# lpylpy0514/VitTracker

Measured on AMD Instinct MI355X. Metric: track() frames/sec per GPU, vit_48_h32, 128px search / 64px template, higher is better.
Workload: dtype f32

## Files before the change

### vittracker_amd/csrc/vt_blocks.h

```cpp
#pragma once
#include <type_traits>
#include "vt_common.h"
#include "vt_bf3.h"

namespace vtb {

constexpr int C = 48;
constexpr int NC = C / 16;
constexpr int HID = 4 * C;
constexpr int NH = HID / 16;
constexpr float LN_EPS = 1e-5f;

constexpr int O_LN1G = 0;
constexpr int O_LN1B = O_LN1G + C;
constexpr int O_WQKV = O_LN1B + C;
constexpr int O_BQKV = O_WQKV + 9 * NC * 256;
constexpr int O_WPROJ = O_BQKV + 3 * C;
constexpr int O_BPROJ = O_WPROJ + NC * NC * 256;
constexpr int O_LN2G = O_BPROJ + C;
constexpr int O_LN2B = O_LN2G + C;
constexpr int O_W1 = O_LN2B + C;
constexpr int O_B1 = O_W1 + NH * NC * 256;
constexpr int O_W2 = O_B1 + HID;
constexpr int O_B2 = O_W2 + NC * NH * 256;
// ... 113 lines not shown
        opa(0, a[0]);
#pragma unroll
        for (int c = 0; c < NCHUNK; ++c) {
            if (c + 1 < NCHUNK) opa(c + 1, a[(c + 1) & 1]);
            if constexpr (SHARED_IS_B) mfma4_shared_b(a[c & 1], ops(c), acc);
            else mfma4_shared_a(ops(c), a[c & 1], acc);
        }
    }
}

template <int NT, int NW, int TPW, bool WLDS, bool BAL = false, bool ZC = false, bool BF3 = false, bool A3 = false>
__global__ __launch_bounds__(NW * 64, (NW == 5 && !WLDS) ? 3 : 1) void blocks_kernel(const float* __restrict__ tokens,
                                                         const float* __restrict__ params,
                                                         float* __restrict__ feat,
                                                         float* __restrict__ resid,
                                                         int len_z, int depth_total, int nblocks,
                                                         int dbg_skip_tile,
                                                         unsigned long long* __restrict__ stamps,
                                                         float* __restrict__ zcache,
                                                         int zcache_mode,
                                                         const float* __restrict__ params3,
                                                         unsigned* __restrict__ vlscr) {
    static_assert(NW * TPW >= NT, "tiles must be covered");
    constexpr bool BF3L = BF3 && WLDS, BF3G = BF3 && !WLDS;
    static_assert(!BF3L || (BAL && 2 * NT * NC >= W3_FC2_TILES - WBUF_TILES), "BF3 with staging: written for the balanced frame form; fc2's third output tile is staged in the K / V area");
    static_assert(!BAL || (WLDS && TPW == 1 && NW == 2 * (NT - 1)), "balanced variant: NT-1 owners + NT-1 guests");
    static_assert(!A3 || BF3, "A3: written for the three-piece forms");
    constexpr bool VP3 = A3 && BF3L;
    constexpr bool VP2L = A3 && BF3G;
    constexpr int KP_T16 = W3_FC1_OT16, VP_PAIRS = NT / 2, VP_T16 = VP_PAIRS * 3 * 64 + (NT & 1) * 3 * 32;
    constexpr int KV_UNITS = A3 ? NT * KP_T16 + (VP3 ? NC * VP_T16 : NC * NT * 64) : 2 * NT * NC * 64;
    constexpr int L = NT * 16;
    constexpr int NOWN = BAL ? NT - 1 : NT;
    constexpr int GT = NT - 1;
    extern __shared__ __attribute__((aligned(16))) float lds[];
    f4* Kimg = reinterpret_cast<f4*>(lds);
    f4* Vimg = Kimg + (A3 ? NT * KP_T16 : NT * NC * 64);
    opnd* const Ko = reinterpret_cast<opnd*>(Kimg);
    opnd* const Vo = reinterpret_cast<opnd*>(Vimg);
    f4* Wa = Kimg + KV_UNITS;
    constexpr int WA_TILES = BF3L ? W3_FC1_TILES : WBUF_TILES;
    f4* Wb = Wa + WA_TILES * 64;
    float* Sp = reinterpret_cast<float*>(WLDS ? Wb + WBUF_TILES * 64 : Wa);
    f4* const Gx = reinterpret_cast<f4*>(Sp + small_floats(depth_total));
    f4* Qg = A3 ? Wb + W3_PROJ_TILES * 64 : Gx;
    f4* Pg = Qg + (A3 ? KP_T16 : NC * 64);
    f4* Dg = A3 ? Gx : Pg + 4 * NC * 64;
    float* Mg = reinterpret_cast<float*>(A3 ? Pg + 4 * NC * 64 : Dg + NC * 64);
    int* gflag = A3 ? reinterpret_cast<int*>(Dg + NC * 64) : reinterpret_cast<int*>(Mg + 4 * 2 * 64);
    f4* Pg2 = A3 ? Wa + W3_QKV_TILES * 64 : Pg;
    static_assert(!A3 || (W3_PROJ_TILES * 64 + KP_T16 + 4 * NC * 64 + 4 * 2 * 64 / 4 <= WBUF_TILES * 64 && W3_QKV_TILES * 64 + 4 * NC * 64 <= W3_FC1_TILES * 64),
                  "A3: the exchange areas fit behind proj's / qkv's image");

    const int b = blockIdx.x;
    const int lane = threadIdx.x & 63;
    const int w = __builtin_amdgcn_readfirstlane(threadIdx.x >> 6);
    const int tok = lane & 15, q = lane >> 4;
    const int g = w - (NT - 1);
    const float scale = 0.14433756729740643f;
    constexpr float SCALE_LOG2E = 0.14433756729740643f * 1.4426950408889634f;
    const int guest_prio = dbg_skip_tile == -3 ? 0 : 1;
    const bool fine = dbg_skip_tile == -2 || dbg_skip_tile <= -100;
    if (dbg_skip_tile <= -100) dbg_skip_tile = -100 - dbg_skip_tile;
    int nstamp = 0;
    auto stamp = [&]() {
        if (stamps != nullptr) {
            unsigned long long t;
            asm volatile("s_memtime %0\n\ts_waitcnt lgkmcnt(0)" : "=s"(t)::"memory");
            if (lane == 0) stamps[((size_t)b * NW + w) * 64 + nstamp] = t;
            ++nstamp;
        }
    };
    auto fstamp = [&]() { if (fine) stamp(); };
    stamp();
    auto stage_img = [&](f4* dst, int off, int ntiles, int blk_of) {
        if constexpr (VT_IS_F16)
            stage_tiles(dst, reinterpret_cast<const float*>(reinterpret_cast<const _Float16*>(params3) + (size_t)blk_of * BLOCK_STRIDE + off), (ntiles + 1) / 2, w, NW, lane);
        else
            stage_tiles(dst, params + (size_t)blk_of * BLOCK_STRIDE + off, ntiles, w, NW, lane);
    };
    if constexpr (BF3L) stage_tiles(Wa, params3 + (W3_FC1_TILES + W3_FC2_TILES) * 256, W3_QKV_TILES, w, NW, lane);
    else if constexpr (WLDS) stage_img(Wa, O_WQKV, 9 * NC, 0);
    for (int i = threadIdx.x; 4 * i < small_floats(depth_total); i += NW * 64)
        st4(Sp + 4 * i, ld4(params + small_src(4 * i, depth_total)));

    f4 x[TPW][NC];
#pragma unroll
    for (int i = 0; i < TPW; ++i) {
        const int T = w + NW * i;
        if (T < NOWN && T != dbg_skip_tile) {
            const float* src = tokens + ((size_t)b * L + 16 * T + tok) * C + 4 * q;
#pragma unroll
            for (int c = 0; c < NC; ++c) x[i][c] = ld4(src + 16 * c);
        }
    }
    f4 x4[NC];
    if constexpr (BAL) {
        if (w >= NOWN) {
            const float* src = tokens + ((size_t)b * L + 16 * GT + tok) * C + 4 * q;
#pragma unroll
            for (int c = 0; c < NC; ++c) x4[c] = ld4(src + 16 * c);
        }
        if (threadIdx.x == 0) *gflag = 0;
        if (w >= NOWN && guest_prio > 0) __builtin_amdgcn_s_setprio(2);
    }
    barrier_publish<WLDS>();

    const int lane_k = lane;
    for (int blk = 0; blk < nblocks; ++blk) {
        int lane_s = lane_k;
        if constexpr (BF3) asm volatile("" : "+v"(lane_s));
        const int lane = lane_s, tok = lane & 15, q = lane >> 4;
        const float* __restrict__ P = params + (size_t)blk * BLOCK_STRIDE;
        const float* S = Sp + blk * SMALL_STRIDE;
        const opnd* const Po = VT_IS_F16 ? reinterpret_cast<const opnd*>(reinterpret_cast<const _Float16*>(params3) + (size_t)blk * BLOCK_STRIDE)
                                         : reinterpret_cast<const opnd*>(P);
        const opnd* const Wa_o = reinterpret_cast<const opnd*>(Wa);
        const opnd* const Wb_o = reinterpret_cast<const opnd*>(Wb);
        auto w_qkv = [&](int t) { return WLDS ? Wa_o[t * 64 + lane] : wimg_o(Po + O_WQKV / 4, t, lane); };
        auto w_proj = [&](int t) { return WLDS ? Wb_o[t * 64 + lane] : wimg_o(Po + O_WPROJ / 4, t, lane); };
        auto w_fc1 = [&](int t) { return WLDS ? Wa_o[t * 64 + lane] : wimg_o(Po + O_W1 / 4, t, lane); };
        auto w_fc2 = [&](int t) { return WLDS ? Wb_o[t * 64 + lane] : wimg_o(Po + O_W2 / 4, t, lane); };
        const float* __restrict__ P3 = BF3 ? params3 + (size_t)blk * BLOCK3_STRIDE : nullptr;
        constexpr int PROJ_TILES = NC * NC;
        using vt3::u32x2;
        using vt3::u32x4;
        int lane3 = lane;
        if constexpr (BF3) asm volatile("" : "+v"(lane3));
        const auto Wa3 = BF3L ? lds_lane_base<u32x4>(Wa, 16u * lane3) : nullptr;
        const auto Wa3h = BF3L ? lds_lane_base<u32x2>(Wa, 192u * 16u + 8u * lane3) : nullptr;
        const auto Wb3 = BF3L ? lds_lane_base<u32x4>(Wb, 16u * lane3) : nullptr;
        const auto Wk3 = BF3L ? lds_lane_base<u32x4>(Kimg, 16u * lane3) : nullptr;
        auto w1_load3 = [&](int t, u32x4 (&a0)[3], u32x2 (&a2)[3]) {
#pragma unroll
            for (int pc = 0; pc < 3; ++pc) {
                a0[pc] = Wa3[t * W3_FC1_OT16 + pc * 64];
                a2[pc] = Wa3h[t * W3_FC1_OT16 * 2 + pc * 64];
            }
        };
        auto w2_load3 = [&](int p, u32x4 (&a)[NC][3]) {
#pragma unroll
            for (int ot = 0; ot < NC; ++ot)
#pragma unroll
                for (int pc = 0; pc < 3; ++pc)
                    a[ot][pc] = ot < 2 ? Wb3[((ot * (NH / 2) + p) * 3 + pc) * 64] : Wk3[(p * 3 + pc) * 64];
// ... 64 lines not shown
            }
        };
        auto store_v3 = [&](int T, int ot, f4 r) {
            u32x2 pv[3];
            vt3::split3(r, pv[0], pv[1], pv[2]);
            u32x2* base = reinterpret_cast<u32x2*>(Kimg + NT * KP_T16 + ot * VP_T16);
            if ((NT & 1) && T == NT - 1) {
#pragma unroll
                for (int pc = 0; pc < 3; ++pc) base[VP_PAIRS * 3 * 64 * 2 + pc * 64 + lane3] = pv[pc];
            } else {
#pragma unroll
                for (int pc = 0; pc < 3; ++pc) base[(((T >> 1) * 3 + pc) * 64 + lane3) * 2 + (T & 1)] = pv[pc];
            }
        };
        constexpr int VL_BLK_U4 = NC * VP_PAIRS * 64;
        u32x4* const vl_blk = VP2L ? reinterpret_cast<u32x4*>(vlscr) + ((size_t)b * depth_total + blk) * VL_BLK_U4 : nullptr;
        auto store_v2l = [&](int T, int ot, f4 r) {
            u32x2 pv[3];
            vt3::split3(r, pv[0], pv[1], pv[2]);
            const int pp = T >> 1, hf = T & 1;
#pragma unroll
            for (int pc = 0; pc < 2; ++pc) reinterpret_cast<u32x2*>(Vimg)[((((ot * VP_PAIRS + pp) * 2 + pc) * 64) + lane3) * 2 + hf] = pv[pc];
            reinterpret_cast<u32x2*>(vl_blk)[(((ot * VP_PAIRS + pp) * 64) + lane3) * 2 + hf] = pv[2];
        };
        if constexpr (A3 && BF3L) {
            stage_tiles(Wb, P3 + (W3_FC1_TILES + W3_FC2_TILES + W3_QKV_TILES) * 256, W3_PROJ_TILES, w, NW, lane, blk == 0);
        } else if constexpr (BF3L) {
            stage_tiles(Wb, P + O_WPROJ, PROJ_TILES, w, NW, lane, blk == 0);
        } else if constexpr (WLDS) stage_img(Wb, O_WPROJ, NC * NC, blk);

        f4 qr[TPW][NC];
#pragma unroll
        for (int i = 0; i < TPW; ++i) {
            const int T = w + NW * i;
            const bool z_tile = ZC && blk == 0 && 16 * T < len_z;
            int lane_z = lane;
            if constexpr (ZC) asm volatile("" : "+v"(lane_z));
            f4* const zc = reinterpret_cast<f4*>(zcache) + (((size_t)b * (len_z >> 4) + T) * 3 * NC) * 64 + lane_z;
            if (VT_BLK_OWNERS && T < NOWN && T != dbg_skip_tile && z_tile && zcache_mode == 2) {
#pragma unroll
                for (int ot = 0; ot < NC; ++ot) {
                    qr[i][ot] = zc[ot * 64];
                    if constexpr (VP3) store_v3(T, ot, zc[(2 * NC + ot) * 64]);
                    else if constexpr (VP2L) store_v2l(T, ot, zc[(2 * NC + ot) * 64]);
                    else Vo[(ot * NT + T) * 64 + lane] = to_opnd(zc[(2 * NC + ot) * 64]);
                    if constexpr (!A3) Ko[(T * NC + ot) * 64 + lane] = to_opnd(zc[(NC + ot) * 64]);
                }
                if constexpr (A3) {
                    f4 kr[NC];
#pragma unroll
                    for (int ot = 0; ot < NC; ++ot) kr[ot] = zc[(NC + ot) * 64];
                    store_k3(Kimg + T * KP_T16, kr);
                }
            } else if (VT_BLK_OWNERS && T < NOWN && T != dbg_skip_tile) {
                f4 h[NC];
                layer_norm_plain(x[i], h);
                fstamp();
                if constexpr (BF3) {
                    u32x4 hb[3];
                    u32x2 hc[3];
                    split_h3(h, hb, hc);
                    const u32x4* const Gq = reinterpret_cast<const u32x4*>(P3) + (W3_FC1_TILES + W3_FC2_TILES) * 64;
                    const u32x2* const Gqh = reinterpret_cast<const u32x2*>(Gq);
                    auto wq_load3 = [&](int t, u32x4 (&a0)[3], u32x2 (&a2)[3]) {
                        if constexpr (BF3L) w1_load3(t, a0, a2);
                        else {
#pragma unroll
                            for (int pc = 0; pc < 3; ++pc) {
                                a0[pc] = Gq[t * W3_FC1_OT16 + pc * 64 + lane3];
                                a2[pc] = Gqh[(t * W3_FC1_OT16 + 192) * 2 + pc * 64 + lane3];
                            }
                        }
                    };
                    u32x4 a0[2][3];
                    u32x2 a2[2][3];
                    auto bias_q = [&](int t) { return t < 2 * NC ? ld4(S + S_BQKV + 16 * t + 4 * q) : splat4(S[S_BQKV + 2 * C + 16 * (t % NC) + tok]); };
                    f4 bias[2];
                    f4 kr[NC];
                    wq_load3(0, a0[0], a2[0]);
                    bias[0] = bias_q(0);
#pragma unroll
                    for (int t = 0; t < 3 * NC; ++t) {
                        if (t + 1 < 3 * NC) {
                            wq_load3(t + 1, a0[(t + 1) & 1], a2[(t + 1) & 1]);
                            bias[(t + 1) & 1] = bias_q(t + 1);
                        }
                        const int ot = t % NC;
// ... 26 lines not shown
                        [&](int c, opnd (&a)[2 * NC]) {
#pragma unroll
                            for (int ot = 0; ot < 2 * NC; ++ot) a[ot] = w_qkv(ot * NC + c);
                        },
                        [&](int c) { return h[c]; }, acc);
#pragma unroll
                    for (int ot = 0; ot < NC; ++ot) {
                        qr[i][ot] = acc[ot];
                        Ko[(T * NC + ot) * 64 + lane] = to_opnd(acc[NC + ot]);
                        if (z_tile && zcache_mode == 1) { zc[ot * 64] = acc[ot]; zc[(NC + ot) * 64] = acc[NC + ot]; }
                    }
                }
                fstamp();
                {
                    f4 acc[NC];
#pragma unroll
                    for (int ot = 0; ot < NC; ++ot) acc[ot] = splat4(S[S_BQKV + 2 * C + 16 * ot + tok]);
                    gemm_stage<NC, NC, false, WLDS>(
                        [&](int c, opnd (&bw)[NC]) {
#pragma unroll
                            for (int ot = 0; ot < NC; ++ot) bw[ot] = w_qkv((2 * NC + ot) * NC + c);
                        },
                        [&](int c) { return h[c]; }, acc);
#pragma unroll
                    for (int ot = 0; ot < NC; ++ot) {
                        Vo[(ot * NT + T) * 64 + lane] = to_opnd(acc[ot]);
                        if (z_tile && zcache_mode == 1) zc[(2 * NC + ot) * 64] = acc[ot];
                    }
                }
                }
            }
        }
        if constexpr (BAL) {
            if (BF3L && VT_BLK_GUESTS && w >= NOWN && g < 3) {
                f4 h[NC];
                layer_norm_plain(x4, h);
                u32x4 hb[3];
                u32x2 hc[3];
                split_h3(h, hb, hc);
                u32x4 a0[NC][3];
                u32x2 a2[NC][3];
#pragma unroll
                for (int j = 0; j < NC; ++j) w1_load3(NC * g + j, a0[j], a2[j]);
                f4 r[NC];
                if (g < 2) {
                    f4 bias[NC];
#pragma unroll
                    for (int j = 0; j < NC; ++j) bias[j] = ld4(S + S_BQKV + 16 * (g * NC + j) + 4 * q);
                    __builtin_amdgcn_sched_barrier(0);
#pragma unroll
                    for (int j = 0; j < NC; ++j) r[j] = tile48(std::false_type{}, a0[j], a2[j], hb, hc, bias[j]);
                    if constexpr (A3) {
                        store_k3(g == 0 ? Qg : Kimg + GT * KP_T16, r);
                    } else {
#pragma unroll
                        for (int j = 0; j < NC; ++j) {
                            if (g == 0) Qg[j * 64 + lane] = r[j];
                            else Ko[(GT * NC + j) * 64 + lane] = to_opnd(r[j]);
                        }
                    }
                } else {
                    f4 bias[NC];
#pragma unroll
                    for (int j = 0; j < NC; ++j) bias[j] = splat4(S[S_BQKV + 2 * C + 16 * j + tok]);
                    __builtin_amdgcn_sched_barrier(0);
#pragma unroll
                    for (int j = 0; j < NC; ++j) r[j] = tile48(std::true_type{}, a0[j], a2[j], hb, hc, bias[j]);
#pragma unroll
                    for (int j = 0; j < NC; ++j) {
                        if constexpr (A3) store_v3(GT, j, r[j]);
                        else Vo[(j * NT + GT) * 64 + lane] = to_opnd(r[j]);
                    }
                }
            } else if (VT_BLK_GUESTS && w >= NOWN && g < 3) {
                f4 h[NC];
                layer_norm_plain(x4, h);
                f4 acc[NC];
                if (g < 2) {
#pragma unroll
                    for (int ot = 0; ot < NC; ++ot) acc[ot] = ld4(S + S_BQKV + 16 * (g * NC + ot) + 4 * q);
                    gemm_stage<NC, NC, true, true>(
                        [&](int c, opnd (&a)[NC]) {
#pragma unroll
                            for (int ot = 0; ot < NC; ++ot) a[ot] = w_qkv((g * NC + ot) * NC + c);
                        },
                        [&](int c) { return h[c]; }, acc);
#pragma unroll
                    for (int ot = 0; ot < NC; ++ot) {
                        if (g == 0) Qg[ot * 64 + lane] = acc[ot];
                        else Ko[(GT * NC + ot) * 64 + lane] = to_opnd(acc[ot]);
                    }
                } else {
#pragma unroll
                    for (int ot = 0; ot < NC; ++ot) acc[ot] = splat4(S[S_BQKV + 2 * C + 16 * ot + tok]);
                    gemm_stage<NC, NC, false, true>(
                        [&](int c, opnd (&bw)[NC]) {
#pragma unroll
                            for (int ot = 0; ot < NC; ++ot) bw[ot] = w_qkv((2 * NC + ot) * NC + c);
                        },
                        [&](int c) { return h[c]; }, acc);
#pragma unroll
                    for (int ot = 0; ot < NC; ++ot) Vo[(ot * NT + GT) * 64 + lane] = to_opnd(acc[ot]);
                }
            }
        }
        stamp();
        if constexpr (VP2L) asm volatile("s_waitcnt vmcnt(0)" ::: "memory");
        barrier_publish<WLDS>();
        stamp();
        if constexpr (BF3L) {
            stage_tiles(Wa, P3, W3_FC1_TILES, w, NW, lane, blk == 0);
        } else if constexpr (WLDS) stage_img(Wa, O_W1, NH * NC, blk);
        const bool last_skip_z = (blk == depth_total - 1) && (resid == nullptr);
#pragma unroll
        for (int i = 0; i < TPW; ++i) {
            const int T = w + NW * i;
            if (A3 && VT_BLK_OWNERS && T < NOWN && T != dbg_skip_tile && !(last_skip_z && 16 * T < len_z)) {
                constexpr int TW[6] = {2, 0, 1, 1, 0, 0}, TX[6] = {0, 2, 1, 0, 1, 0};
                u32x4 qb[3];
                u32x2 qc[3];
                split_h3(qr[i], qb, qc);
                f4 s[NT];
                float m0 = -3.0e38f, m1 = -3.0e38f;
                {
                    constexpr int NB = VP3 ? 2 : 1;
                    u32x4 a0[NB][3];
                    u32x2 a2[NB][3];
                    if (NB == 2) k_load3(0, a0[0], a2[0]);
#pragma unroll
                    for (int J = 0; J < NT; ++J) {
                        if (NB == 2 && J + 1 < NT) k_load3(J + 1, a0[(J + 1) % NB], a2[(J + 1) % NB]);
                        if (NB == 1) k_load3(J, a0[0], a2[0]);
                        __builtin_amdgcn_sched_barrier(0);
                        s[J] = tile48(std::false_type{}, a0[J % NB], a2[J % NB], qb, qc, splat4(0.f));
                        m0 = fmaxf(fmaxf(m0, s[J].x), s[J].y);
                        m1 = fmaxf(fmaxf(m1, s[J].z), s[J].w);
                    }
                }
                fstamp();
                const float m = quad_max(fmaxf(m0, m1));
                const f2 k2 = {SCALE_LOG2E, SCALE_LOG2E}, nm2 = {-m * SCALE_LOG2E, -m * SCALE_LOG2E};
                f2 d0 = {0.f, 0.f}, d1 = {0.f, 0.f};
                f4 o[NC];
                constexpr int NWB = VP3 ? 2 : 1;
                u32x4 wa0[NWB][3];
                u32x2 wa2[NWB][3];
                if constexpr (VP3) {
                    u32x4 pb[VP_PAIRS > 0 ? VP_PAIRS : 1][3];
                    u32x2 po[3], plo[3];
                    u32x4 v[NC][3];
// ... 108 lines not shown
                        const f2 c = __builtin_elementwise_fma(f2{s[J].z, s[J].w}, k2, nm2);
                        const f2 ea = {__builtin_amdgcn_exp2f(a.x), __builtin_amdgcn_exp2f(a.y)};
                        const f2 ec = {__builtin_amdgcn_exp2f(c.x), __builtin_amdgcn_exp2f(c.y)};
                        s[J] = f4{ea.x, ea.y, ec.x, ec.y};
                        d0 += ea;
                        d1 += ec;
                    }
                    const f2 dd = d0 + d1;
                    const float rden = __builtin_amdgcn_rcpf(quad_sum(dd.x + dd.y));
                    fstamp();
#pragma unroll
                    for (int t = 0; t < NC; ++t) o[t] = splat4(0.f);
                    gemm_stage<NT, NC, true, WLDS>(
                        [&](int J, opnd (&a)[NC]) {
#pragma unroll
                            for (int t = 0; t < NC; ++t) a[t] = Vo[(t * NT + J) * 64 + lane];
                        },
                        [&](int J) { return s[J]; }, o);
#pragma unroll
                    for (int t = 0; t < NC; ++t) o[t] = o[t] * splat4(rden);
                }
                fstamp();
                u32x4 ob[3];
                u32x2 oc[3];
                split_h3(o, ob, oc);
#pragma unroll
                for (int ot = 0; ot < NC; ++ot) {
                    if (NWB == 2 && ot + 1 < NC) wp_load3(ot + 1, wa0[(ot + 1) % NWB], wa2[(ot + 1) % NWB]);
                    if (NWB == 1) wp_load3(ot, wa0[0], wa2[0]);
                    __builtin_amdgcn_sched_barrier(0);
                    x[i][ot] = tile48(std::false_type{}, wa0[ot % NWB], wa2[ot % NWB], ob, oc, x[i][ot] + ld4(S + S_BPROJ + 16 * ot + 4 * q));
                    __builtin_amdgcn_sched_barrier(0);
                }
            } else if (!A3 && VT_BLK_OWNERS && T < NOWN && T != dbg_skip_tile && !(last_skip_z && 16 * T < len_z)) {
                f4 s[NT];
                float m0 = -3.0e38f, m1 = -3.0e38f;
                constexpr int JG = 5;
                static_assert(NT % JG == 0, "NT must be a multiple of 5");
#pragma unroll
                for (int j0 = 0; j0 < NT; j0 += JG) {
                    f4 acc[JG];
#pragma unroll
                    for (int j = 0; j < JG; ++j) acc[j] = splat4(0.f);
                    gemm_stage<NC, JG, true, WLDS>(
                        [&](int c, opnd (&a)[JG]) {
#pragma unroll
                            for (int j = 0; j < JG; ++j) a[j] = Ko[((j0 + j) * NC + c) * 64 + lane];
                        },
                        [&](int c) { return qr[i][c]; }, acc);
#pragma unroll
                    for (int j = 0; j < JG; ++j) {
                        s[j0 + j] = acc[j];
                        m0 = fmaxf(fmaxf(m0, acc[j].x), acc[j].y);
                        m1 = fmaxf(fmaxf(m1, acc[j].z), acc[j].w);
                    }
                }
                fstamp();
                const float m = quad_max(fmaxf(m0, m1));
                const f2 k2 = {SCALE_LOG2E, SCALE_LOG2E}, nm2 = {-m * SCALE_LOG2E, -m * SCALE_LOG2E};
                f2 d0 = {0.f, 0.f}, d1 = {0.f, 0.f};
#pragma unroll
                for (int J = 0; J < NT; ++J) {
                    const f2 a = __builtin_elementwise_fma(f2{s[J].x, s[J].y}, k2, nm2);
                    const f2 c = __builtin_elementwise_fma(f2{s[J].z, s[J].w}, k2, nm2);
                    const f2 ea = {__builtin_amdgcn_exp2f(a.x), __builtin_amdgcn_exp2f(a.y)};
                    const f2 ec = {__builtin_amdgcn_exp2f(c.x), __builtin_amdgcn_exp2f(c.y)};
                    s[J] = f4{ea.x, ea.y, ec.x, ec.y};
                    d0 += ea;
                    d1 += ec;
                }
                const f2 dd = d0 + d1;
                const float den = dd.x + dd.y;
                const float rden = __builtin_amdgcn_rcpf(quad_sum(den));
                fstamp();
                f4 o[NC];
#pragma unroll
                for (int t = 0; t < NC; ++t) o[t] = splat4(0.f);
                gemm_stage<NT, NC, true, WLDS>(
                    [&](int J, opnd (&a)[NC]) {
#pragma unroll
                        for (int t = 0; t < NC; ++t) a[t] = Vo[(t * NT + J) * 64 + lane];
                    },
                    [&](int J) { return s[J]; }, o);
#pragma unroll
                for (int t = 0; t < NC; ++t) o[t] = o[t] * splat4(rden);
                fstamp();
#pragma unroll
                for (int ot = 0; ot < NC; ++ot) x[i][ot] = x[i][ot] + ld4(S + S_BPROJ + 16 * ot + 4 * q);
                gemm_stage<NC, NC, true, WLDS>(
                    [&](int c, opnd (&a)[NC]) {
#pragma unroll
                        for (int ot = 0; ot < NC; ++ot) a[ot] = w_proj(ot * NC + c);
                    },
                    [&](int c) { return o[c]; }, x[i]);
            }
        }
        if constexpr (BAL) {
            if (VT_BLK_GUESTS && w >= NOWN) {
                auto attn_part = [&](auto njc, int J0) {
                    constexpr int NJ = decltype(njc)::value;
                    f4 qv[NC];
#pragma unroll
                    for (int c = 0; c < NC; ++c) qv[c] = Qg[c * 64 + lane];
                    f4 sc[NJ];
#pragma unroll
                    for (int j = 0; j < NJ; ++j) sc[j] = splat4(0.f);
                    gemm_stage<NC, NJ, true, true>(
                        [&](int c, opnd (&a)[NJ]) {
#pragma unroll
                            for (int j = 0; j < NJ; ++j) a[j] = Ko[((J0 + j) * NC + c) * 64 + lane];
                        },
                        [&](int c) { return qv[c]; }, sc);
                    float m0 = -3.0e38f, m1 = -3.0e38f;
#pragma unroll
                    for (int j = 0; j < NJ; ++j) {
                        m0 = fmaxf(fmaxf(m0, sc[j].x), sc[j].y);
                        m1 = fmaxf(fmaxf(m1, sc[j].z), sc[j].w);
                    }
                    const float mraw = quad_max(fmaxf(m0, m1));
                    const float m = mraw * scale;
                    const f2 k2 = {SCALE_LOG2E, SCALE_LOG2E}, nm2 = {-mraw * SCALE_LOG2E, -mraw * SCALE_LOG2E};
                    f2 d0 = {0.f, 0.f}, d1 = {0.f, 0.f};
#pragma unroll
                    for (int j = 0; j < NJ; ++j) {
                        const f2 a = __builtin_elementwise_fma(f2{sc[j].x, sc[j].y}, k2, nm2);
                        const f2 c = __builtin_elementwise_fma(f2{sc[j].z, sc[j].w}, k2, nm2);
                        const f2 ea = {__builtin_amdgcn_exp2f(a.x), __builtin_amdgcn_exp2f(a.y)};
                        const f2 ec = {__builtin_amdgcn_exp2f(c.x), __builtin_amdgcn_exp2f(c.y)};
                        sc[j] = f4{ea.x, ea.y, ec.x, ec.y};
                        d0 += ea;
                        d1 += ec;
// ... 327 lines not shown
                for (int e = 0; e < 6; ++e) {
                    if (t < NH) {
                        accB = vt3::mma16(a2[t & 1][TW[e]], hc[TX[e]], accB);
                        accA = vt3::mma(a0[t & 1][TW[e]], hb[TX[e]], accA);
                    }
                    if (t > 0) {
                        if (e < 5) gstage(e);
                        else gfinish(t - 1);
                    }
                    __builtin_amdgcn_sched_barrier(0);
                }
                prev = accA + accB;
            }
        };
        auto mlp_second3 = [&](int i, int hi) {
            constexpr int NP = NH / 2;
            constexpr int TW[6] = {2, 0, 1, 1, 0, 0}, TX[6] = {0, 2, 1, 0, 1, 0};
            u32x4 a[2][NC][3];
            w2_load3(0, a[0]);
#pragma unroll
            for (int p = 0; p < NP; ++p) {
                if (p + 1 < NP) w2_load3(p + 1, a[(p + 1) & 1]);
                __builtin_amdgcn_sched_barrier(0);
#pragma unroll
                for (int e = 0; e < 6; ++e)
#pragma unroll
                    for (int ot = 0; ot < NC; ++ot) x[i][ot] = vt3::mma(a[p & 1][ot][TW[e]], hq[hi][p][TX[e]], x[i][ot]);
                if (p == 1 || p == 3) fstamp();
            }
        };
        if constexpr (BF3L) {
#pragma unroll
            for (int i = 0; i < TPW; ++i) {
                const int T = w + NW * i;
                if (VT_BLK_OWNERS && T < NOWN && T != dbg_skip_tile && !(last_skip_z && 16 * T < len_z)) mlp_first3(i, i);
            }
            u32x2 gq[NC][3];
            if (VT_BLK_GUESTS && w >= NOWN) {
#pragma unroll
                for (int ot = 0; ot < NC; ++ot) x4[ot] = x4[ot] + ld4(S + S_BPROJ + 16 * ot + 4 * q) + Dg[ot * 64 + lane];
                f4 h[NC];
                layer_norm_plain(x4, h);
#pragma unroll
                for (int ot = 0; ot < NC; ++ot) x4[ot] = x4[ot] + ld4(S + S_B2 + 16 * ot + 4 * q);
                u32x4 hb[3];
                u32x2 hc[3];
                split_h3(h, hb, hc);
                u32x4 a0[NC][3];
                u32x2 a2[NC][3];
#pragma unroll
                for (int j = 0; j < NC; ++j) w1_load3(NC * g + j, a0[j], a2[j]);
                f4 acc[NC];
#pragma unroll
                for (int j = 0; j < NC; ++j) acc[j] = ld4(S + S_B1 + 16 * (NC * g + j) + 4 * q);
                __builtin_amdgcn_sched_barrier(0);
                fc1_terms3(std::integral_constant<int, NC>{}, a0, a2, hb, hc, acc);
#pragma unroll
                for (int j = 0; j < NC; ++j) vt3::split3(gelu4(acc[j]), gq[j][0], gq[j][1], gq[j][2]);
            }
                stamp();
            barrier_publish<true>();
            if (blk + 1 < nblocks) stage_tiles(Wa, P3 + BLOCK3_STRIDE + (W3_FC1_TILES + W3_FC2_TILES) * 256, W3_QKV_TILES, w, NW, lane, false);
            stamp();
#pragma unroll
            for (int i = 0; i < TPW; ++i) {
                const int T = w + NW * i;
                if (VT_BLK_OWNERS && T < NOWN && T != dbg_skip_tile && !(last_skip_z && 16 * T < len_z)) mlp_second3(i, i);
            }
            if (VT_BLK_GUESTS && w >= NOWN) {
                const bool odd = g & 1;
                const int p_full = (3 * g + (odd ? 1 : 0)) >> 1, p_half = (3 * g + (odd ? 0 : 2)) >> 1;
                u32x4 bf[3];
                u32x2 bh[3];
#pragma unroll
                for (int pc = 0; pc < 3; ++pc) {
                    bf[pc] = odd ? u32x4{gq[1][pc].x, gq[1][pc].y, gq[2][pc].x, gq[2][pc].y} : u32x4{gq[0][pc].x, gq[0][pc].y, gq[1][pc].x, gq[1][pc].y};
                    bh[pc] = odd ? gq[0][pc] : gq[2][pc];
                }
                u32x4 af[NC][3];
                u32x2 ah[NC][3];
                w2_load3(p_full, af);
                {
                    const unsigned hoff = 16u * lane3 + (odd ? 8u : 0u) + (unsigned)p_half * (3u * 64u * 16u);
                    const auto Wb3h = lds_lane_base<u32x2>(Wb, hoff);
                    const auto Wk3h = lds_lane_base<u32x2>(Kimg, hoff);
#pragma unroll
                    for (int ot = 0; ot < NC; ++ot)
#pragma unroll
                        for (int pc = 0; pc < 3; ++pc)
                            ah[ot][pc] = ot < 2 ? Wb3h[((ot * (NH / 2)) * 3 + pc) * 64 * 2] : Wk3h[pc * 64 * 2];
                }
                f4 part[NC], partB[NC];
#pragma unroll
                for (int ot = 0; ot < NC; ++ot) part[ot] = partB[ot] = splat4(0.f);
                __builtin_amdgcn_sched_barrier(0);
                constexpr int TW[6] = {2, 0, 1, 1, 0, 0}, TX[6] = {0, 2, 1, 0, 1, 0};
#pragma unroll
                for (int half = 0; half < 2; ++half)
#pragma unroll
                    for (int k = 0; k < 2; ++k)
#pragma unroll
                        for (int t3 = 0; t3 < 3; ++t3)
#pragma unroll
                            for (int ot = 0; ot < NC; ++ot) {
                                const int e = 3 * half + t3;
                                if (k == 0) partB[ot] = vt3::mma16(ah[ot][TW[e]], bh[TX[e]], partB[ot]);
                                else part[ot] = vt3::mma(af[ot][TW[e]], bf[TX[e]], part[ot]);
                            }
#pragma unroll
                for (int ot = 0; ot < NC; ++ot) part[ot] = part[ot] + partB[ot];
#pragma unroll
                for (int ot = 0; ot < NC; ++ot) Pg2[(g * NC + ot) * 64 + lane] = part[ot];
            }
        } else if constexpr (WLDS) {
#pragma unroll
            for (int i = 0; i < TPW; ++i) {
                const int T = w + NW * i;
                if (VT_BLK_OWNERS && T < NOWN && T != dbg_skip_tile && !(last_skip_z && 16 * T < len_z)) mlp_first(i, i);
            }
            f4 ghid[NC];
            if constexpr (BAL) {
                if (VT_BLK_GUESTS && w >= NOWN) {
#pragma unroll
                    for (int ot = 0; ot < NC; ++ot) x4[ot] = x4[ot] + ld4(S + S_BPROJ + 16 * ot + 4 * q) + Dg[ot * 64 + lane];
                    f4 h[NC];
                    layer_norm_plain(x4, h);
#pragma unroll
                    for (int ot = 0; ot < NC; ++ot) x4[ot] = x4[ot] + ld4(S + S_B2 + 16 * ot + 4 * q);
#pragma unroll
                    for (int j = 0; j < NC; ++j) ghid[j] = ld4(S + S_B1 + 16 * (NC * g + j) + 4 * q);
                    gemm_stage<NC, NC, true, true>(
                        [&](int c, opnd (&a)[NC]) {
#pragma unroll
                            for (int j = 0; j < NC; ++j) a[j] = w_fc1((NC * g + j) * NC + c);
                        },
                        [&](int c) { return h[c]; }, ghid);
#pragma unroll
                    for (int j = 0; j < NC; ++j)
                        ghid[j] = gelu4(ghid[j]);
                }
            }
            stamp();
            barrier_publish<WLDS>();
            if (blk + 1 < nblocks) stage_img(Wa, O_WQKV, 9 * NC, blk + 1);
            stamp();
#pragma unroll
            for (int i = 0; i < TPW; ++i) {
                const int T = w + NW * i;
                if (VT_BLK_OWNERS && T < NOWN && T != dbg_skip_tile && !(last_skip_z && 16 * T < len_z)) mlp_second(i, i);
            }
            if constexpr (BAL) {
                if (VT_BLK_GUESTS && w >= NOWN) {
                    f4 part[NC];
#pragma unroll
                    for (int ot = 0; ot < NC; ++ot) part[ot] = splat4(0.f);
                    gemm_stage<NC, NC, true, true>(
                        [&](int cc, opnd (&a)[NC]) {
#pragma unroll
                            for (int ot = 0; ot < NC; ++ot) a[ot] = w_fc2(ot * NH + NC * g + cc);
                        },
                        [&](int cc) { return ghid[cc]; }, part);
#pragma unroll
                    for (int ot = 0; ot < NC; ++ot) Pg[(g * NC + ot) * 64 + lane] = part[ot];
                }
            }
        } else {
#pragma unroll
            for (int i = 0; i < TPW; ++i) {
                const int T = w + NW * i;
                if (BF3G && T < NT && T != dbg_skip_tile && !(last_skip_z && 16 * T < len_z)) {
                    const u32x4* const G1 = reinterpret_cast<const u32x4*>(P3);
                    const u32x2* const G1h = reinterpret_cast<const u32x2*>(P3);
                    const u32x4* const G2 = G1 + W3_FC1_TILES * 64;
                    auto g1_load3 = [&](int t, u32x4 (&a0)[3], u32x2 (&a2)[3]) {
#pragma unroll
                        for (int pc = 0; pc < 3; ++pc) {
                            a0[pc] = G1[t * W3_FC1_OT16 + pc * 64 + lane3];
                            a2[pc] = G1h[(t * W3_FC1_OT16 + 192) * 2 + pc * 64 + lane3];
                        }
                    };
                    f4 h[NC];
                    layer_norm_plain(x[i], h);
                    u32x4 hb[3];
                    u32x2 hc[3];
                    split_h3(h, hb, hc);
// ... 47 lines not shown
                    f4 hd[NH];
                    constexpr int G6 = 6;
#pragma unroll
                    for (int g = 0; g < NH; g += G6) {
                        f4 acc[G6];
#pragma unroll
                        for (int j = 0; j < G6; ++j) acc[j] = ld4(S + S_B1 + 16 * (g + j) + 4 * q);
#pragma unroll
                        for (int c = 0; c < NC; ++c) {
                            opnd a[G6];
#pragma unroll
                            for (int j = 0; j < G6; ++j) a[j] = w_fc1((g + j) * NC + c);
                            mfma4_shared_b(a, h[c], acc);
                        }
#pragma unroll
                        for (int j = 0; j < G6; ++j)
                            hd[g + j] = gelu4(acc[j]);
                    }
#pragma unroll
                    for (int ot = 0; ot < NC; ++ot) x[i][ot] = x[i][ot] + ld4(S + S_B2 + 16 * ot + 4 * q);
#pragma unroll
                    for (int c = 0; c < NH; ++c) {
                        opnd a[NC];
#pragma unroll
                        for (int ot = 0; ot < NC; ++ot) a[ot] = w_fc2(ot * NH + c);
                        mfma4_shared_b(a, hd[c], x[i]);
                    }
                }
            }
        }
        stamp();
        if constexpr (WLDS) barrier_publish<true>();
        if constexpr (BAL) {
            if (w >= NOWN) {
#pragma unroll
                for (int k = 0; k < 4; ++k)
#pragma unroll
                    for (int ot = 0; ot < NC; ++ot) x4[ot] = x4[ot] + Pg2[(k * NC + ot) * 64 + lane];
            }
        }
    }

    stamp();
    const float* PF = Sp + depth_total * SMALL_STRIDE;
    int lane_e = lane_k;
    if constexpr (BF3) asm volatile("" : "+v"(lane_e));
    const int tok_e = lane_e & 15, q_e = lane_e >> 4;
    const int Lx = L - len_z;
    if constexpr (BAL) {
        if (g == 0) {
            if (resid != nullptr) {
                float* dst = resid + ((size_t)b * L + 16 * GT + tok_e) * C + 4 * q_e;
#pragma unroll
                for (int c = 0; c < NC; ++c) st4(dst + 16 * c, x4[c]);
            }
            f4 h[NC];
            layer_norm_img(x4, h, PF, PF + C, q_e);
            float* dst = feat + ((size_t)b * Lx + (16 * GT - len_z) + tok_e) * C + 4 * q_e;
#pragma unroll
            for (int c = 0; c < NC; ++c) st4(dst + 16 * c, h[c]);
        }
    }
#pragma unroll
    for (int i = 0; i < TPW; ++i) {
        const int T = w + NW * i;
        if (T < NOWN) {
            if (resid != nullptr) {
                float* dst = resid + ((size_t)b * L + 16 * T + tok_e) * C + 4 * q_e;
#pragma unroll
                for (int c = 0; c < NC; ++c) st4(dst + 16 * c, x[i][c]);
            }
            if (16 * T >= len_z) {
                f4 h[NC];
                layer_norm_img(x[i], h, PF, PF + C, q_e);
                float* dst = feat + ((size_t)b * Lx + (16 * T - len_z) + tok_e) * C + 4 * q_e;
#pragma unroll
                for (int c = 0; c < NC; ++c) st4(dst + 16 * c, h[c]);
            }
        }
    }
}

}
```

Measured before the change: 3.263 million.

## Assign template tile to guest waves so z-cache and last-block skip apply

When the template is a single 16-token tile, the balanced variant now gives the guest group tile 0 instead of the last search tile, and shifts owners by one tile. The guests can then read their QKV from the template cache in block 0 and skip their whole block in the last layer when residuals are not needed. Before, only the owners benefited from these skips, which left the guest group on the critical path. This adds runtime tile-offset logic and, in the non-BF3 case, aliases the guest registers onto x[0], which raises correctness and register-pressure risk.

Result: faster. 3.385 million, median of 6 (+3.8%).

```diff
diff --git a/vittracker_amd/csrc/vt_blocks.h b/vittracker_amd/csrc/vt_blocks.h
--- a/vittracker_amd/csrc/vt_blocks.h
+++ b/vittracker_amd/csrc/vt_blocks.h
@@ -169,7 +169,8 @@
     constexpr int KV_UNITS = A3 ? NT * KP_T16 + (VP3 ? NC * VP_T16 : NC * NT * 64) : 2 * NT * NC * 64;
     constexpr int L = NT * 16;
     constexpr int NOWN = BAL ? NT - 1 : NT;
-    constexpr int GT = NT - 1;
+    const int toff = (BAL && len_z == 16) ? 1 : 0;
+    const int GT = toff ? 0 : NT - 1;
     extern __shared__ __attribute__((aligned(16))) float lds[];
     f4* Kimg = reinterpret_cast<f4*>(lds);
     f4* Vimg = Kimg + (A3 ? NT * KP_T16 : NT * NC * 64);
@@ -224,14 +225,15 @@
     f4 x[TPW][NC];
 #pragma unroll
     for (int i = 0; i < TPW; ++i) {
-        const int T = w + NW * i;
-        if (T < NOWN && T != dbg_skip_tile) {
+        const int T = w + NW * i + toff;
+        if (T - toff < NOWN && T != dbg_skip_tile) {
             const float* src = tokens + ((size_t)b * L + 16 * T + tok) * C + 4 * q;
 #pragma unroll
             for (int c = 0; c < NC; ++c) x[i][c] = ld4(src + 16 * c);
         }
     }
-    f4 x4[NC];
+    f4 x4s[NC];
+    f4 (&x4)[NC] = (BAL && !BF3) ? x[0] : x4s;
     if constexpr (BAL) {
         if (w >= NOWN) {
             const float* src = tokens + ((size_t)b * L + 16 * GT + tok) * C + 4 * q;
@@ -248,6 +250,9 @@
         int lane_s = lane_k;
         if constexpr (BF3) asm volatile("" : "+v"(lane_s));
         const int lane = lane_s, tok = lane & 15, q = lane >> 4;
+        const bool last_skip_z = (blk == depth_total - 1) && (resid == nullptr);
+        const bool guest_skip = BAL && last_skip_z && toff != 0;
+        const bool zg_tile = BAL && ZC && blk == 0 && toff != 0;
         const float* __restrict__ P = params + (size_t)blk * BLOCK_STRIDE;
         const float* S = Sp + blk * SMALL_STRIDE;
         const opnd* const Po = VT_IS_F16 ? reinterpret_cast<const opnd*>(reinterpret_cast<const _Float16*>(params3) + (size_t)blk * BLOCK_STRIDE)
@@ -378,12 +383,12 @@
         f4 qr[TPW][NC];
 #pragma unroll
         for (int i = 0; i < TPW; ++i) {
-            const int T = w + NW * i;
+            const int T = w + NW * i + toff;
             const bool z_tile = ZC && blk == 0 && 16 * T < len_z;
             int lane_z = lane;
             if constexpr (ZC) asm volatile("" : "+v"(lane_z));
             f4* const zc = reinterpret_cast<f4*>(zcache) + (((size_t)b * (len_z >> 4) + T) * 3 * NC) * 64 + lane_z;
-            if (VT_BLK_OWNERS && T < NOWN && T != dbg_skip_tile && z_tile && zcache_mode == 2) {
+            if (VT_BLK_OWNERS && T - toff < NOWN && T != dbg_skip_tile && z_tile && zcache_mode == 2) {
 #pragma unroll
                 for (int ot = 0; ot < NC; ++ot) {
                     qr[i][ot] = zc[ot * 64];
@@ -398,7 +403,7 @@
                     for (int ot = 0; ot < NC; ++ot) kr[ot] = zc[(NC + ot) * 64];
                     store_k3(Kimg + T * KP_T16, kr);
                 }
-            } else if (VT_BLK_OWNERS && T < NOWN && T != dbg_skip_tile) {
+            } else if (VT_BLK_OWNERS && T - toff < NOWN && T != dbg_skip_tile) {
                 f4 h[NC];
                 layer_norm_plain(x[i], h);
                 fstamp();
@@ -491,76 +496,116 @@
             }
         }
         if constexpr (BAL) {
-            if (BF3L && VT_BLK_GUESTS && w >= NOWN && g < 3) {
-                f4 h[NC];
-                layer_norm_plain(x4, h);
-                u32x4 hb[3];
-                u32x2 hc[3];
-                split_h3(h, hb, hc);
-                u32x4 a0[NC][3];
-                u32x2 a2[NC][3];
-#pragma unroll
-                for (int j = 0; j < NC; ++j) w1_load3(NC * g + j, a0[j], a2[j]);
+            auto zc_guest = [&]() {
+                int lane_z = lane;
+                asm volatile("" : "+v"(lane_z));
+                return reinterpret_cast<f4*>(zcache) + ((size_t)b * 3 * NC + NC * g) * 64 + lane_z;
+            };
+            auto with_gt = [&](auto f) {
+                if (toff) f(std::integral_constant<int, 0>{});
+                else f(std::integral_constant<int, NT - 1>{});
+            };
+            const bool guest_qkv = VT_BLK_GUESTS && w >= NOWN && g < 3 && !(guest_skip && g == 0);
+            if (BF3L && guest_qkv) {
                 f4 r[NC];
-                if (g < 2) {
-                    f4 bias[NC];
-#pragma unroll
-                    for (int j = 0; j < NC; ++j) bias[j] = ld4(S + S_BQKV + 16 * (g * NC + j) + 4 * q);
-                    __builtin_amdgcn_sched_barrier(0);
-#pragma unroll
-                    for (int j = 0; j < NC; ++j) r[j] = tile48(std::false_type{}, a0[j], a2[j], hb, hc, bias[j]);
-                    if constexpr (A3) {
-                        store_k3(g == 0 ? Qg : Kimg + GT * KP_T16, r);
+                if (zg_tile && zcache_mode == 2) {
+                    const f4* const zc = zc_guest();
+#pragma unroll
+                    for (int j = 0; j < NC; ++j) r[j] = zc[j * 64];
+                } else {
+                    f4 h[NC];
+                    layer_norm_plain(x4, h);
+                    u32x4 hb[3];
+                    u32x2 hc[3];
+                    split_h3(h, hb, hc);
+                    u32x4 a0[NC][3];
+                    u32x2 a2[NC][3];
+#pragma unroll
+                    for (int j = 0; j < NC; ++j) w1_load3(NC * g + j, a0[j], a2[j]);
+                    if (g < 2) {
+                        f4 bias[NC];
+#pragma unroll
+                        for (int j = 0; j < NC; ++j) bias[j] = ld4(S + S_BQKV + 16 * (g * NC + j) + 4 * q);
+                        __builtin_amdgcn_sched_barrier(0);
+#pragma unroll
+                        for (int j = 0; j < NC; ++j) r[j] = tile48(std::false_type{}, a0[j], a2[j], hb, hc, bias[j]);
                     } else {
+                        f4 bias[NC];
+#pragma unroll
+                        for (int j = 0; j < NC; ++j) bias[j] = splat4(S[S_BQKV + 2 * C + 16 * j + tok]);
+                        __builtin_amdgcn_sched_barrier(0);
+#pragma unroll
+                        for (int j = 0; j < NC; ++j) r[j] = tile48(std::true_type{}, a0[j], a2[j], hb, hc, bias[j]);
+                    }
+                    if (zg_tile && zcache_mode == 1) {
+                        f4* const zc = zc_guest();
+#pragma unroll
+                        for (int j = 0; j < NC; ++j) zc[j * 64] = r[j];
+                    }
+                }
+                with_gt([&](auto gt) {
+                    constexpr int GTc = decltype(gt)::value;
+                    if (g < 2) {
+                        if constexpr (A3) {
+                            store_k3(g == 0 ? Qg : Kimg + GTc * KP_T16, r);
+                        } else {
+#pragma unroll
+                            for (int j = 0; j < NC; ++j) {
+                                if (g == 0) Qg[j * 64 + lane] = r[j];
+                                else Ko[(GTc * NC + j) * 64 + lane] = to_opnd(r[j]);
+                            }
+                        }
+                    } else {
 #pragma unroll
                         for (int j = 0; j < NC; ++j) {
-                            if (g == 0) Qg[j * 64 + lane] = r[j];
-                            else Ko[(GT * NC + j) * 64 + lane] = to_opnd(r[j]);
+                            if constexpr (A3) store_v3(GTc, j, r[j]);
+                            else Vo[(j * NT + GTc) * 64 + lane] = to_opnd(r[j]);
                         }
                     }
+                });
+            } else if (guest_qkv) {
+                f4 acc[NC];
+                if (zg_tile && zcache_mode == 2) {
+                    const f4* const zc = zc_guest();
+#pragma unroll
+                    for (int ot = 0; ot < NC; ++ot) acc[ot] = zc[ot * 64];
                 } else {
-                    f4 bias[NC];
-#pragma unroll
-                    for (int j = 0; j < NC; ++j) bias[j] = splat4(S[S_BQKV + 2 * C + 16 * j + tok]);
-                    __builtin_amdgcn_sched_barrier(0);
-#pragma unroll
-                    for (int j = 0; j < NC; ++j) r[j] = tile48(std::true_type{}, a0[j], a2[j], hb, hc, bias[j]);
-#pragma unroll
-                    for (int j = 0; j < NC; ++j) {
-                        if constexpr (A3) store_v3(GT, j, r[j]);
-                        else Vo[(j * NT + GT) * 64 + lane] = to_opnd(r[j]);
-                    }
-                }
-            } else if (VT_BLK_GUESTS && w >= NOWN && g < 3) {
-                f4 h[NC];
-                layer_norm_plain(x4, h);
-                f4 acc[NC];
-                if (g < 2) {
-#pragma unroll
-                    for (int ot = 0; ot < NC; ++ot) acc[ot] = ld4(S + S_BQKV + 16 * (g * NC + ot) + 4 * q);
-                    gemm_stage<NC, NC, true, true>(
-                        [&](int c, opnd (&a)[NC]) {
-#pragma unroll
-                            for (int ot = 0; ot < NC; ++ot) a[ot] = w_qkv((g * NC + ot) * NC + c);
-                        },
-                        [&](int c) { return h[c]; }, acc);
+                    f4 h[NC];
+                    layer_norm_plain(x4, h);
+                    if (g < 2) {
+#pragma unroll
+                        for (int ot = 0; ot < NC; ++ot) acc[ot] = ld4(S + S_BQKV + 16 * (g * NC + ot) + 4 * q);
+                        gemm_stage<NC, NC, true, true>(
+                            [&](int c, opnd (&a)[NC]) {
+#pragma unroll
+                                for (int ot = 0; ot < NC; ++ot) a[ot] = w_qkv((g * NC + ot) * NC + c);
+                            },
+                            [&](int c) { return h[c]; }, acc);
+                    } else {
+#pragma unroll
+                        for (int ot = 0; ot < NC; ++ot) acc[ot] = splat4(S[S_BQKV + 2 * C + 16 * ot + tok]);
+                        gemm_stage<NC, NC, false, true>(
+                            [&](int c, opnd (&bw)[NC]) {
+#pragma unroll
+                                for (int ot = 0; ot < NC; ++ot) bw[ot] = w_qkv((2 * NC + ot) * NC + c);
+                            },
+                            [&](int c) { return h[c]; }, acc);
+                    }
+                    if (zg_tile && zcache_mode == 1) {
+                        f4* const zc = zc_guest();
+#pragma unroll
+                        for (int ot = 0; ot < NC; ++ot) zc[ot * 64] = acc[ot];
+                    }
+                }
+                with_gt([&](auto gt) {
+                    constexpr int GTc = decltype(gt)::value;
 #pragma unroll
                     for (int ot = 0; ot < NC; ++ot) {
                         if (g == 0) Qg[ot * 64 + lane] = acc[ot];
-                        else Ko[(GT * NC + ot) * 64 + lane] = to_opnd(acc[ot]);
-                    }
-                } else {
-#pragma unroll
-                    for (int ot = 0; ot < NC; ++ot) acc[ot] = splat4(S[S_BQKV + 2 * C + 16 * ot + tok]);
-                    gemm_stage<NC, NC, false, true>(
-                        [&](int c, opnd (&bw)[NC]) {
-#pragma unroll
-                            for (int ot = 0; ot < NC; ++ot) bw[ot] = w_qkv((2 * NC + ot) * NC + c);
-                        },
-                        [&](int c) { return h[c]; }, acc);
-#pragma unroll
-                    for (int ot = 0; ot < NC; ++ot) Vo[(ot * NT + GT) * 64 + lane] = to_opnd(acc[ot]);
-                }
+                        else if (g == 1) Ko[(GTc * NC + ot) * 64 + lane] = to_opnd(acc[ot]);
+                        else Vo[(ot * NT + GTc) * 64 + lane] = to_opnd(acc[ot]);
+                    }
+                });
             }
         }
         stamp();
@@ -570,11 +615,10 @@
         if constexpr (BF3L) {
             stage_tiles(Wa, P3, W3_FC1_TILES, w, NW, lane, blk == 0);
         } else if constexpr (WLDS) stage_img(Wa, O_W1, NH * NC, blk);
-        const bool last_skip_z = (blk == depth_total - 1) && (resid == nullptr);
 #pragma unroll
         for (int i = 0; i < TPW; ++i) {
-            const int T = w + NW * i;
-            if (A3 && VT_BLK_OWNERS && T < NOWN && T != dbg_skip_tile && !(last_skip_z && 16 * T < len_z)) {
+            const int T = w + NW * i + toff;
+            if (A3 && VT_BLK_OWNERS && T - toff < NOWN && T != dbg_skip_tile && !(last_skip_z && 16 * T < len_z)) {
                 constexpr int TW[6] = {2, 0, 1, 1, 0, 0}, TX[6] = {0, 2, 1, 0, 1, 0};
                 u32x4 qb[3];
                 u32x2 qc[3];
@@ -749,7 +793,7 @@
                     x[i][ot] = tile48(std::false_type{}, wa0[ot % NWB], wa2[ot % NWB], ob, oc, x[i][ot] + ld4(S + S_BPROJ + 16 * ot + 4 * q));
                     __builtin_amdgcn_sched_barrier(0);
                 }
-            } else if (!A3 && VT_BLK_OWNERS && T < NOWN && T != dbg_skip_tile && !(last_skip_z && 16 * T < len_z)) {
+            } else if (!A3 && VT_BLK_OWNERS && T - toff < NOWN && T != dbg_skip_tile && !(last_skip_z && 16 * T < len_z)) {
                 f4 s[NT];
                 float m0 = -3.0e38f, m1 = -3.0e38f;
                 constexpr int JG = 5;
@@ -813,7 +857,7 @@
             }
         }
         if constexpr (BAL) {
-            if (VT_BLK_GUESTS && w >= NOWN) {
+            if (VT_BLK_GUESTS && w >= NOWN && !guest_skip) {
                 auto attn_part = [&](auto njc, int J0) {
                     constexpr int NJ = decltype(njc)::value;
                     f4 qv[NC];
@@ -1207,11 +1251,11 @@
         if constexpr (BF3L) {
 #pragma unroll
             for (int i = 0; i < TPW; ++i) {
-                const int T = w + NW * i;
-                if (VT_BLK_OWNERS && T < NOWN && T != dbg_skip_tile && !(last_skip_z && 16 * T < len_z)) mlp_first3(i, i);
+                const int T = w + NW * i + toff;
+                if (VT_BLK_OWNERS && T - toff < NOWN && T != dbg_skip_tile && !(last_skip_z && 16 * T < len_z)) mlp_first3(i, i);
             }
             u32x2 gq[NC][3];
-            if (VT_BLK_GUESTS && w >= NOWN) {
+            if (VT_BLK_GUESTS && w >= NOWN && !guest_skip) {
 #pragma unroll
                 for (int ot = 0; ot < NC; ++ot) x4[ot] = x4[ot] + ld4(S + S_BPROJ + 16 * ot + 4 * q) + Dg[ot * 64 + lane];
                 f4 h[NC];
@@ -1239,10 +1283,10 @@
             stamp();
 #pragma unroll
             for (int i = 0; i < TPW; ++i) {
-                const int T = w + NW * i;
-                if (VT_BLK_OWNERS && T < NOWN && T != dbg_skip_tile && !(last_skip_z && 16 * T < len_z)) mlp_second3(i, i);
-            }
-            if (VT_BLK_GUESTS && w >= NOWN) {
+                const int T = w + NW * i + toff;
+                if (VT_BLK_OWNERS && T - toff < NOWN && T != dbg_skip_tile && !(last_skip_z && 16 * T < len_z)) mlp_second3(i, i);
+            }
+            if (VT_BLK_GUESTS && w >= NOWN && !guest_skip) {
                 const bool odd = g & 1;
                 const int p_full = (3 * g + (odd ? 1 : 0)) >> 1, p_half = (3 * g + (odd ? 0 : 2)) >> 1;
                 u32x4 bf[3];
@@ -1290,12 +1334,12 @@
         } else if constexpr (WLDS) {
 #pragma unroll
             for (int i = 0; i < TPW; ++i) {
-                const int T = w + NW * i;
-                if (VT_BLK_OWNERS && T < NOWN && T != dbg_skip_tile && !(last_skip_z && 16 * T < len_z)) mlp_first(i, i);
+                const int T = w + NW * i + toff;
+                if (VT_BLK_OWNERS && T - toff < NOWN && T != dbg_skip_tile && !(last_skip_z && 16 * T < len_z)) mlp_first(i, i);
             }
             f4 ghid[NC];
             if constexpr (BAL) {
-                if (VT_BLK_GUESTS && w >= NOWN) {
+                if (VT_BLK_GUESTS && w >= NOWN && !guest_skip) {
 #pragma unroll
                     for (int ot = 0; ot < NC; ++ot) x4[ot] = x4[ot] + ld4(S + S_BPROJ + 16 * ot + 4 * q) + Dg[ot * 64 + lane];
                     f4 h[NC];
@@ -1321,11 +1365,11 @@
             stamp();
 #pragma unroll
             for (int i = 0; i < TPW; ++i) {
-                const int T = w + NW * i;
-                if (VT_BLK_OWNERS && T < NOWN && T != dbg_skip_tile && !(last_skip_z && 16 * T < len_z)) mlp_second(i, i);
+                const int T = w + NW * i + toff;
+                if (VT_BLK_OWNERS && T - toff < NOWN && T != dbg_skip_tile && !(last_skip_z && 16 * T < len_z)) mlp_second(i, i);
             }
             if constexpr (BAL) {
-                if (VT_BLK_GUESTS && w >= NOWN) {
+                if (VT_BLK_GUESTS && w >= NOWN && !guest_skip) {
                     f4 part[NC];
 #pragma unroll
                     for (int ot = 0; ot < NC; ++ot) part[ot] = splat4(0.f);
@@ -1439,7 +1483,7 @@
         stamp();
         if constexpr (WLDS) barrier_publish<true>();
         if constexpr (BAL) {
-            if (w >= NOWN) {
+            if (w >= NOWN && !guest_skip) {
 #pragma unroll
                 for (int k = 0; k < 4; ++k)
 #pragma unroll
@@ -1461,17 +1505,19 @@
 #pragma unroll
                 for (int c = 0; c < NC; ++c) st4(dst + 16 * c, x4[c]);
             }
-            f4 h[NC];
-            layer_norm_img(x4, h, PF, PF + C, q_e);
-            float* dst = feat + ((size_t)b * Lx + (16 * GT - len_z) + tok_e) * C + 4 * q_e;
-#pragma unroll
-            for (int c = 0; c < NC; ++c) st4(dst + 16 * c, h[c]);
+            if (16 * GT >= len_z) {
+                f4 h[NC];
+                layer_norm_img(x4, h, PF, PF + C, q_e);
+                float* dst = feat + ((size_t)b * Lx + (16 * GT - len_z) + tok_e) * C + 4 * q_e;
+#pragma unroll
+                for (int c = 0; c < NC; ++c) st4(dst + 16 * c, h[c]);
+            }
         }
     }
 #pragma unroll
     for (int i = 0; i < TPW; ++i) {
-        const int T = w + NW * i;
-        if (T < NOWN) {
+        const int T = w + NW * i + toff;
+        if (T - toff < NOWN) {
             if (resid != nullptr) {
                 float* dst = resid + ((size_t)b * L + 16 * T + tok_e) * C + 4 * q_e;
 #pragma unroll
```
